# 10XGenomics/vartrix

Hardware: NVIDIA H100
Metric: reads_sw_scored_per_sec (higher is better)
Workload: dtype int16x2

## Files before the change

### include/vartrix_b200.h

```cpp
#ifndef VARTRIX_B200_H
#define VARTRIX_B200_H

#include <stdint.h>

#ifdef __cplusplus
extern "C" {
#endif

#define VTX_ABI_VERSION 2

#define VTX_OK             0
#define VTX_E_INVALID     (-1)
#define VTX_E_CUDA        (-2)
#define VTX_E_NOMEM       (-3)
#define VTX_E_UNSUPPORTED (-4)
#define VTX_E_STATE       (-5)
#define VTX_E_NCCL        (-6)

#define VTX_MODE_CONSENSUS 0
#define VTX_MODE_COVERAGE  1
#define VTX_MODE_ALT_FRAC  2

#define VTX_NO_CB   0xFFFFFFFFu
#define VTX_NO_UMI  0xFFFFFFFFFFFFFFFFull
// ... 162 lines not shown
int         vtx_submit_bam(vtx_ctx* ctx, const vtx_bam_shard* shard);
int         vtx_bam_metrics_get(vtx_ctx* ctx, vtx_bam_metrics* out);
int         vtx_set_min_base_quality(vtx_ctx* ctx, uint32_t min_q);
int         vtx_bam_low_base_quality(vtx_ctx* ctx, uint64_t* out);

uint64_t    vtx_pack_cb(const uint8_t* s, uint32_t len);

typedef struct vtx_timing {
    float h2d_ms;
    float prep_ms;
    float sw_ms;
    float post_ms;
    uint64_t n_pairs;
    uint64_t sw_launches;
    uint64_t total_launches;
} vtx_timing;
int         vtx_last_timing(vtx_ctx* ctx, vtx_timing* out);
int         vtx_last_tile_counts(vtx_ctx* ctx, uint32_t* out, uint32_t n_out);

int         vtx_comm_unique_id(uint8_t id_out[128]);
int         vtx_comm_init(vtx_ctx* ctx, const uint8_t id[128], int32_t rank, int32_t n_ranks);
int         vtx_gather(vtx_ctx* ctx, vtx_result* out);
#define VTX_GATHER_ALL (-1)
int         vtx_gather_start(vtx_ctx* ctx, int32_t root);
int         vtx_gather_wait(vtx_ctx* ctx, vtx_result* out);

#ifdef __cplusplus
}
#endif
#endif
// ... 1 lines not shown
```

### vartrix_b200/_capi.py

```python
from __future__ import annotations

import ctypes as C
import os

_HERE = os.path.dirname(os.path.abspath(__file__))
LIB_PATH = os.environ.get("VTX_LIB") or os.path.join(_HERE, "lib", "libvartrix_b200.so")

VTX_OK = 0
MODE_CONSENSUS, MODE_COVERAGE, MODE_ALT_FRAC = 0, 1, 2
MODES = {"consensus": MODE_CONSENSUS, "coverage": MODE_COVERAGE, "alt_frac": MODE_ALT_FRAC}
NO_CB = 0xFFFFFFFF
NO_UMI = 0xFFFFFFFFFFFFFFFF
F_KEEP_SCORES = 1
F_NO_SPLIT = 2
F_VALUES_ONLY = 4
F_NO_FOLD = 8
F_NAME_KEYS = 16

SYMBOLS = [
    "vtx_abi_version", "vtx_create", "vtx_destroy", "vtx_last_error", "vtx_host_alloc", "vtx_host_free",
    "vtx_set_barcodes", "vtx_submit", "vtx_submit_device", "vtx_submit_device_ex", "vtx_finish",
    "vtx_finish_device", "vtx_fetch", "vtx_sync", "vtx_wait_copies", "vtx_score_pairs", "vtx_pack_umi", "vtx_last_timing", "vtx_last_tile_counts",
    "vtx_comm_unique_id", "vtx_comm_init", "vtx_gather", "vtx_gather_start", "vtx_gather_wait",
    "vtx_submit2", "vtx_submit2_device", "vtx_pack_cb", "vtx_bgzf_inflate", "vtx_submit_bam", "vtx_bam_metrics_get",
# ... 61 lines not shown
                ("num_duplicates", C.c_uint64), ("num_not_useful", C.c_uint64)]


class Metrics(C.Structure):
    _fields_ = [("num_not_cell_bc", C.c_uint64), ("num_non_umi", C.c_uint64), ("num_scored", C.c_uint64)]


class Result(C.Structure):
    _fields_ = [("n", C.c_uint64), ("row", C.c_void_p), ("col", C.c_void_p), ("ref_cnt", C.c_void_p),
                ("alt_cnt", C.c_void_p), ("unk_cnt", C.c_void_p), ("val", C.c_void_p), ("val2", C.c_void_p),
                ("metrics", Metrics)]


class Timing(C.Structure):
    _fields_ = [("h2d_ms", C.c_float), ("prep_ms", C.c_float), ("sw_ms", C.c_float), ("post_ms", C.c_float),
                ("n_pairs", C.c_uint64), ("sw_launches", C.c_uint64), ("total_launches", C.c_uint64)]


_lib = None


def load():
    global _lib
    if _lib is not None:
        return _lib
    if not os.path.exists(LIB_PATH):
        raise RuntimeError(f"{LIB_PATH} is missing: run `make` (or __graft_entry__.build()) first; "
                           "vartrix_b200 has no CPU fallback")
    L = C.CDLL(LIB_PATH)
    L.vtx_abi_version.restype = C.c_int
    L.vtx_create.restype = C.c_int
# ... 58 lines not shown
```

### vartrix_b200/csrc/vtx_api.cu

```cuda
#include "../../include/vartrix_b200.h"
#include "vtx_pipeline.cuh"
#include "vtx_sw.cuh"
#include "vtx_sw_band.cuh"
#include "vtx_inflate.cuh"
#include "vtx_stage.cuh"

#include <nvtx3/nvToolsExt.h>

#include <algorithm>
#include <array>
#include <cstdarg>
#include <cstddef>
#include <cstdio>
#include <cstring>
#include <string>
#include <thread>
#include <vector>

using namespace vtx;

namespace {

thread_local std::string g_create_error;

// ... 88 lines not shown
    DBuf inf_comp, inf_out, inf_desc, inf_status;
    bool inflate_attr_set = false;
    StageSlot sslot[2];
    uint64_t n_bam_submits = 0;
    cudaStream_t stage_stream = nullptr;
    DBuf bam_metrics;
    uint32_t min_base_quality = 0;
    DBuf stage_sums;
    HostBuf h_stage;
    uint32_t bc_cap = 0, n_barcodes = 0;
    bool have_barcodes = false;

    InSlot slot[2];
    uint64_t n_submits = 0;
    cudaStream_t copy_stream = nullptr;
    DBuf read_col, keep, pidx, scan_sums, pair_read, pair_col, pair_umi, pair_locus, pair_start, tcount, tstart,
        pair_first, pair_cslot, pair_uslot, cslot_col, cslot_locus, uslot_cslot, ccnt, ucnt, keep2, oidx, tile_counters,
        scratch, pair_scores, d_metrics, d_res_n, big_list, slot_scratch;
    DBuf res[kResArrays];
    size_t res_cap = 0;
    size_t res_ub = 0;
    bool finished = true;
    HostResults h_res;
    HostBuf h_scalars;
    uint64_t last_n = 0;
    vtx_metrics last_metrics{};

    cudaStream_t fetch_stream = nullptr;
    HostBuf h_cum;
    unsigned long long* d_cum = nullptr;
    std::vector<TimeRec> trecs;
    size_t trec_used = 0;
    bool timing_valid = false;
    uint32_t last_tiles_nl = 0;
    bool last_tiles_valid = false;
    uint64_t t_pairs = 0;

    void* comm = nullptr;
    int rank = 0, n_ranks = 1;
    HostResults g_host;
    DBuf g_dev[kResArrays];
    DBuf g_counts;
    cudaStream_t comm_stream = nullptr;
    cudaEvent_t ev_counts = nullptr, ev_gather = nullptr, ev_results = nullptr;
    HostBuf h_counts;
    bool gather_pending = false;
    bool gather_guard = false;
    vtx_result g_out{};
};

namespace {
// ... 164 lines not shown
    return launch_sw(ctx, vtx_k_sw_pairs<CLS>, TileClass<CLS>::THREADS,
                     sw_warp_bytes<CLS>(a.mcap, a.multi) * (TileClass<CLS>::THREADS / 32), a, launches,
                     "SW kernel class", CLS);
}
template <int SCLS> int launch_sw_split(vtx_ctx* ctx, const SwArgs& a, uint64_t* launches)
{
    return launch_sw(ctx, vtx_k_sw_split<SCLS>, SplitClass<SCLS>::THREADS,
                     split_warp_bytes<SCLS>(a.mcap) * (SplitClass<SCLS>::THREADS / 32), a, launches,
                     "split SW kernel", SCLS);
}
template <int W, int S, bool SHARED> int launch_sw_fold(vtx_ctx* ctx, const SwArgs& a, uint64_t* launches)
{
    return launch_sw(ctx, vtx_k_sw_fold<W, S, SHARED>, W * 32, fold_cta_bytes<W, S>(), a, launches, "folded SW kernel", -1);
}

int run_sw(vtx_ctx* ctx, const DevBatch& b, uint32_t n_pairs_ub, const uint32_t* pair_slot, uint32_t* counters,
           uint32_t* pair_scores, uint64_t* launches, uint64_t* sw_launches, TimeRec* tr)
{
    const uint32_t nl = b.n_loci;
    ENS(ctx->tcount, size_t(kNumClasses) * (nl + 1) * 4);
    ENS(ctx->tstart, size_t(kNumClasses) * (nl + 1) * 4);
    ENS(ctx->tile_counters, 64);
    const SwAllow allow = sw_allow(ctx, b.max_read_len, b.max_hap_len);
    vtx_k_locus_prep<<<blocks_for(uint64_t(nl) * 32, 256), 256, 0, ctx->stream>>>(
        nl, b.hap, b.ref_off, b.ref_len, b.alt_off, b.alt_len, P<uint32_t>(ctx->pair_start), P<uint32_t>(ctx->pair_read), b.read_len,
        0, allow.split, allow.multi, allow.fold, b.max_read_len, b.max_hap_len, P<unsigned long long>(ctx->d_metrics) + 4,
        P<uint32_t>(ctx->tcount));
    ++*launches;
    vtx_k_scan_rows<<<kNumClasses, kScanThreads, 0, ctx->stream>>>(P<uint32_t>(ctx->tcount), P<uint32_t>(ctx->tstart), nl, nl + 1);
    ++*launches;
    CK(cudaGetLastError());
    CK(cudaMemsetAsync(ctx->tile_counters.p, 0, 64, ctx->stream));
    ctx->last_tiles_nl = nl;
    ctx->last_tiles_valid = true;
    if (tr) CK(cudaEventRecord(tr->ev[EV_PREP], ctx->stream));

    SwArgs a{};
    a.hap_bytes = b.hap; a.ref_off = b.ref_off; a.ref_len = b.ref_len; a.alt_off = b.alt_off; a.alt_len = b.alt_len;
    a.read_nib = b.read_nib; a.read_off = b.read_off; a.read_len = b.read_len;
    a.pair_read = P<uint32_t>(ctx->pair_read); a.pair_start = P<uint32_t>(ctx->pair_start);
    a.n_loci = nl; a.pair_slot = pair_slot; a.counters = counters; a.pair_scores = pair_scores;
    a.min_score = ctx->cfg.min_score;
    int mcap = int(std::min<uint32_t>(b.max_read_len, kFastMaxRead));
    mcap = std::max(2, (mcap + 1) & ~1);
    a.mcap = mcap;
    a.k64k = 65536u;
    a.one = 1u;
    a.multi = allow.multi;
    a.max_hap = b.max_hap_len;

    uint64_t before = *launches;
    if (ctx->cfg.band_mode == VTX_BAND_MODEL) {
        BandArgs ba{};
        ba.sw = a; ba.n_pairs_ub = n_pairs_ub; ba.k = ctx->cfg.band_k; ba.w = ctx->cfg.band_w;
        ba.max_read = std::max<uint32_t>(b.max_read_len, 8); ba.max_hap = std::max<uint32_t>(b.max_hap_len, 8);
// ... 86 lines not shown
    }
    ctx->res_cap = ncap;
    return VTX_OK;
}

int process_batch(vtx_ctx* ctx, const DevBatch& b, TimeRec* tr)
{
    const uint64_t nc = b.n_cand;
    const uint32_t nl = b.n_loci, nr = b.n_reads;
    const int use_umi = ctx->cfg.use_umi ? 1 : 0;
    uint64_t launches = 0, sw_launches = 0;
    cudaStream_t st = ctx->stream;

    if (ctx->finished) {
        CK(cudaMemsetAsync(ctx->d_res_n.p, 0, 8, st));
        CK(cudaMemsetAsync(ctx->d_metrics.p, 0, 48, st));
        ctx->res_ub = 0;
        ctx->finished = false;
    }
    int rc = grow_results(ctx, ctx->res_ub + nc);
    if (rc) return rc;

    const size_t ncp = size_t(nc) + 1;
    ENS(ctx->read_col, size_t(nr ? nr : 1) * 4);
    ENS(ctx->keep, ncp * 4); ENS(ctx->pidx, ncp * 4);
    ENS(ctx->pair_read, ncp * 4); ENS(ctx->pair_col, ncp * 4);
    if (use_umi) ENS(ctx->pair_umi, ncp * 8);
    ENS(ctx->pair_start, size_t(nl + 1) * 4);
    ENS(ctx->pair_first, ncp);
    ENS(ctx->pair_cslot, ncp * 4); ENS(ctx->cslot_col, ncp * 4); ENS(ctx->cslot_locus, ncp * 4);
    ENS(ctx->ccnt, ncp * 16);
// ... 865 lines not shown
}

int vtx_wait_copies(vtx_ctx* ctx)
{
    if (!ctx) return VTX_E_INVALID;
    CK(cudaSetDevice(ctx->device));
    CK(cudaStreamSynchronize(ctx->copy_stream));
    return VTX_OK;
}

static int finish_scalars(vtx_ctx* ctx)
{
    CK(cudaSetDevice(ctx->device));
    uint64_t* hs = ctx->h_scalars.as<uint64_t>();
    CK(cudaMemcpyAsync(hs, ctx->d_res_n.p, 8, cudaMemcpyDeviceToHost, ctx->stream));
    CK(cudaMemcpyAsync(hs + 1, ctx->d_metrics.p, 48, cudaMemcpyDeviceToHost, ctx->stream));
    CK(cudaStreamSynchronize(ctx->stream));
    const uint64_t violated = ctx->finished ? 0 : hs[5], band_overflow = ctx->finished ? 0 : hs[6];
    ctx->last_n = ctx->finished ? 0 : hs[0];
    ctx->last_metrics.num_not_cell_bc = ctx->finished ? 0 : hs[1];
    ctx->last_metrics.num_non_umi = ctx->finished ? 0 : hs[2];
    ctx->last_metrics.num_scored = ctx->finished ? 0 : hs[3];
    ctx->t_pairs = ctx->last_metrics.num_scored;
    ctx->finished = true;
    if (band_overflow)
        return set_err(ctx, VTX_E_UNSUPPORTED, "band model: %llu alignments had more k-mer hits than the work buffers hold (reads x windows too large); "
                                               "they were scored with the full matrix", (unsigned long long)band_overflow);
    if (violated)
        return set_err(ctx, VTX_E_INVALID, "%llu loci of a device batch exceeded the bounds given to vtx_submit_device(_ex) (longest read / widest "
                                           "haplotype window); they were skipped, the result is incomplete", (unsigned long long)violated);
    return VTX_OK;
}

int vtx_finish_device(vtx_ctx* ctx, vtx_result* out)
{
    Nvtx nvtx_range("vtx_finish_device");
    if (!ctx || !out) return VTX_E_INVALID;
    int rc = finish_scalars(ctx);
// ... 78 lines not shown
    if (!ctx || !t) return VTX_E_INVALID;
    if (!ctx->timing_valid || ctx->trec_used == 0) return set_err(ctx, VTX_E_STATE, "no finished submit to time");
    CK(cudaSetDevice(ctx->device));
    memset(t, 0, sizeof(*t));
    for (size_t i = 0; i < ctx->trec_used; ++i) {
        TimeRec& r = ctx->trecs[i];
        CK(cudaEventSynchronize(r.ev[EV_POST]));
        float ms = 0;
        if (r.had_h2d) { CK(cudaEventElapsedTime(&ms, r.ev[EV_START], r.ev[EV_H2D])); t->h2d_ms += ms; }
        CK(cudaEventElapsedTime(&ms, r.ev[EV_C0], r.ev[EV_PREP])); t->prep_ms += ms;
        CK(cudaEventElapsedTime(&ms, r.ev[EV_PREP], r.ev[EV_SW])); t->sw_ms += ms;
        CK(cudaEventElapsedTime(&ms, r.ev[EV_SW], r.ev[EV_POST])); t->post_ms += ms;
        t->sw_launches += r.sw_launches; t->total_launches += r.launches;
    }
    t->n_pairs = ctx->t_pairs;
    return VTX_OK;
}

int vtx_score_pairs(vtx_ctx* ctx, const vtx_batch* hb, uint64_t n_pairs, const uint32_t* pair_read,
                    const uint32_t* pair_locus, int16_t* ref_score, int16_t* alt_score)
{
    Nvtx nvtx_range("vtx_score_pairs");
    if (!ctx) return VTX_E_INVALID;
    if (!hb) return set_err(ctx, VTX_E_INVALID, "batch is NULL");
    BatchView hv0 = view_of(hb); hv0.n_cand = 0; hv0.cand_read = nullptr;
    int rc = validate_batch(ctx, hv0);
    if (rc) return rc;
    if (n_pairs >= 0xFFFFFFF0ull) return set_err(ctx, VTX_E_INVALID, "too many pairs");
    if (n_pairs && (!pair_read || !pair_locus || !ref_score || !alt_score)) return set_err(ctx, VTX_E_INVALID, "NULL pair arrays");
    DevBatch d{};
// ... 225 lines not shown
```

### vartrix_b200/csrc/vtx_pipeline.cuh

```cuda
#pragma once
#include <cstdint>
#include <cuda_runtime.h>
#include "vtx_sw.cuh"
#include "vtx_sw_split.cuh"
#include "vtx_sw_fold.cuh"

namespace vtx {

constexpr uint32_t kNoCb = 0xFFFFFFFFu;
constexpr uint64_t kNoUmi = 0xFFFFFFFFFFFFFFFFull;
constexpr uint32_t kInvalid = 0xFFFFFFFFu;

__host__ __device__ inline uint64_t fnv1a64(const uint8_t* p, uint32_t n)
{
    uint64_t h = 1469598103934665603ull;
    for (uint32_t i = 0; i < n; ++i) { h ^= p[i]; h *= 1099511628211ull; }
    return h;
}

struct BarcodeTable {
    const int32_t* slot;
    uint32_t cap_mask;
    const uint8_t* bytes;
    const uint32_t* off;
// ... 158 lines not shown
{
    const uint32_t l = blockIdx.x * blockDim.x + threadIdx.x;
    if (l <= n_loci) pair_start[l] = pidx[cand_start[l]];
}

__global__ void vtx_k_pair_start_explicit(uint32_t n_loci, uint32_t n_pairs, const uint32_t* __restrict__ pair_locus,
                                          uint32_t* __restrict__ pair_start)
{
    const uint32_t l = blockIdx.x * blockDim.x + threadIdx.x;
    if (l > n_loci) return;
    uint32_t lo = 0, hi = n_pairs;
    while (lo < hi) { const uint32_t mid = (lo + hi) >> 1; if (pair_locus[mid] < l) lo = mid + 1; else hi = mid; }
    pair_start[l] = lo;
}

__global__ void vtx_k_locus_prep(uint32_t n_loci, const uint8_t* __restrict__ hap_bytes,
                                 const uint32_t* __restrict__ ref_off, const uint32_t* __restrict__ ref_len,
                                 const uint32_t* __restrict__ alt_off, const uint32_t* __restrict__ alt_len,
                                 const uint32_t* __restrict__ pair_start, const uint32_t* __restrict__ pair_read,
                                 const uint32_t* __restrict__ read_len, int force_slow, int allow_split, int allow_multi, int allow_fold,
                                 uint32_t max_read, uint32_t max_hap, unsigned long long* __restrict__ bounds_violated,
                                 uint32_t* __restrict__ tcount )
{
    const uint32_t l = (blockIdx.x * blockDim.x + threadIdx.x) >> 5;
    const int lane = threadIdx.x & 31;
    if (l >= n_loci) return;
    const uint32_t nr = ref_len[l], na = alt_len[l];
    const uint8_t* rh = hap_bytes + ref_off[l];
    const uint8_t* ah = hap_bytes + alt_off[l];
    bool exotic = false;
    auto is_exotic = [](uint8_t b) {
        return b == '=' || b == 'M' || b == 'R' || b == 'S' || b == 'V' || b == 'W' || b == 'Y' || b == 'H' ||
               b == 'K' || b == 'D' || b == 'B' || b == 'N';
    };
    for (uint32_t j = lane; j < nr; j += 32) exotic |= is_exotic(rh[j]);
    for (uint32_t j = lane; j < na; j += 32) exotic |= is_exotic(ah[j]);
    exotic = __any_sync(0xffffffffu, exotic);
    bool same = nr >= uint32_t(kSplitP) && na >= uint32_t(kSplitP);
    if (same) for (uint32_t j = lane; j < uint32_t(kSplitP); j += 32) same &= (rh[j] == ah[j]);
    same = __all_sync(0xffffffffu, same);
    bool fold = same && allow_fold && min(nr, na) > uint32_t(2 * kFoldP) && max(nr, na) <= uint32_t(2 * kFoldP + kFoldMaxMid);
    if (fold) for (uint32_t j = lane; j < uint32_t(kFoldP); j += 32) fold &= (rh[nr - 1 - j] == ah[na - 1 - j]);
    fold = __all_sync(0xffffffffu, fold);
    uint32_t longest = 0;
    for (uint32_t p = pair_start[l] + lane; p < pair_start[l + 1]; p += 32) longest = max(longest, read_len[pair_read[p]]);
    longest = __reduce_max_sync(0xffffffffu, longest);
    fold = fold && longest <= uint32_t(kFoldMaxRead);
    if (lane != 0) return;
    const uint32_t nmax = max(nr, na);
    if (longest > max_read || nmax > max_hap) {
        atomicAdd(bounds_violated, 1ull);
#pragma unroll
        for (int c = 0; c < kNumClasses; ++c) tcount[size_t(c) * (n_loci + 1) + l] = 0u;
        return;
    }
    int cls = kSlowClass;
    if (!exotic && !force_slow) {
#pragma unroll
        for (int c = kNumFastClasses - 1; c >= 0; --c) if (nmax <= uint32_t(class_max_n(c))) cls = c;
        if (cls == kSlowClass && allow_multi) cls = kMultiClass;
        if (same && allow_split) {
#pragma unroll
            for (int c = kNumSplitClasses - 1; c >= 0; --c) if (nmax <= uint32_t(split_max_n(c))) cls = kSplitClass0 + c;
        }
        if (fold) cls = kFoldClass;
    }
    const uint32_t np = pair_start[l + 1] - pair_start[l];
#pragma unroll
    for (int c = 0; c < kNumClasses; ++c) {
        const uint32_t ppw = (c == kSlowClass) ? uint32_t(kSlowPairsPerWarp) : (c == kFoldClass ? uint32_t(kFoldPPW) : (c > kSlowClass ? uint32_t(kSplitPPW) : 4u));
        tcount[size_t(c) * (n_loci + 1) + l] = (c == cls) ? (np + ppw - 1) / ppw : 0u;
    }
}

constexpr int kSlotThreads = 128;
constexpr int kSlotChunk = 1024;
constexpr uint32_t kSlotSmallMax = 2048;
constexpr int kSlotBigThreads = 1024;
constexpr int kSlotBigWords = 7;
__global__ void __launch_bounds__(kSlotThreads) vtx_k_slots(
    uint32_t n_loci, const uint32_t* __restrict__ pair_start, const uint32_t* __restrict__ pair_col,
    const uint64_t* __restrict__ pair_umi, int use_umi, uint8_t* __restrict__ pair_first,
// ... 326 lines not shown
```

### vartrix_b200/csrc/vtx_sw.cuh

```cuda
#pragma once
#include <cstdint>
#include <cuda_runtime.h>

namespace vtx {

constexpr int kMatch = 1, kMismatch = -5, kGapOpen = -5, kGapExtend = -1;
constexpr int kGoe = kGapOpen + kGapExtend;

__host__ __device__ constexpr uint32_t pack2(int lo, int hi)
{
    return (uint32_t(uint16_t(int16_t(hi))) << 16) | uint32_t(uint16_t(int16_t(lo)));
}
constexpr int kBias = 16384;
constexpr uint32_t kGE2 = pack2(kGapExtend, kGapExtend);
constexpr uint32_t kBIAS2 = pack2(kBias, kBias);
constexpr uint32_t kGOE2 = pack2(kBias + kGoe, kBias + kGoe);
constexpr uint32_t kNEG2 = pack2(0, 0);
constexpr uint32_t kGoeAdd = (uint32_t(uint16_t(int16_t(kGoe - 1))) << 16) | uint32_t(uint16_t(int16_t(kGoe)));
#ifndef VTX_SW_FUSE
#define VTX_SW_FUSE 1
#endif
#ifndef VTX_SW_HADD
#define VTX_SW_HADD 0
#endif
// ... 42 lines not shown
template <> struct TileClass<3> { static constexpr int LPP = 8, C = 40, CS = 44, THREADS = 384, MINB = 1; };
constexpr int kMultiClass = 3;
constexpr int kMultiMaxRead = 256;
__host__ __device__ constexpr int class_max_n(int cls)
{
    return cls == 0 ? 208 : cls == 1 ? 232 : cls == 2 ? 256 : cls == 3 ? 320 : 0x7fffffff;
}
constexpr int kSlowPairsPerWarp = 16;

struct SwArgs {
    const uint8_t* hap_bytes;
    const uint32_t* ref_off; const uint32_t* ref_len; const uint32_t* alt_off; const uint32_t* alt_len;
    const uint8_t* read_nib; const uint64_t* read_off; const uint32_t* read_len;
    const uint32_t* pair_read;
    const uint32_t* pair_start;
    const uint32_t* tile_start;
    uint32_t n_loci;
    uint32_t* tile_counter;
    const uint32_t* pair_slot;
    uint32_t* counters;
    uint32_t* pair_scores;
    int32_t min_score;
    int32_t mcap;
    uint32_t k64k;
    uint32_t one;
    int32_t multi;
    uint32_t* scratch;
    uint32_t max_hap;
};

// ... 4 lines not shown
__device__ __forceinline__ uint32_t nib_code(uint32_t nib)
{
    return (0x4444444344424104ull >> (nib * 4)) & 0xF;
}

__device__ __forceinline__ uint32_t upper_locus(const uint32_t* __restrict__ a, uint32_t n, uint32_t v)
{
    uint32_t lo = 0, hi = n;
    while (hi - lo > 1) {
        uint32_t mid = (lo + hi) >> 1;
        if (__ldg(a + mid) <= v) lo = mid; else hi = mid;
    }
    return lo;
}

__device__ __forceinline__ void call_and_scatter(const SwArgs& a, uint32_t pair, uint32_t packed)
{
    const int ref_score = int(int16_t(packed & 0xFFFF)), alt_score = int(int16_t(packed >> 16));
    if (a.pair_scores) a.pair_scores[pair] = pack2(ref_score, alt_score);
    if (!a.pair_slot) return;
    if (ref_score < a.min_score && alt_score < a.min_score) return;
    const uint32_t k = ref_score > alt_score ? 0u : (alt_score > ref_score ? 1u : 2u);
    atomicAdd(a.counters + size_t(a.pair_slot[pair]) * 4 + k, 1u);
}

template <int CLS>
__host__ __device__ constexpr size_t sw_warp_bytes(int mcap, int multi)
{
    using TC = TileClass<CLS>;
    constexpr int PPW = 32 / TC::LPP, RS = TC::LPP * TC::CS;
    const int bnd_stride = (CLS == kMultiClass && multi) ? mcap + 8 : 0;
    const size_t codes_bytes = (size_t(PPW) * (mcap + 2 * TC::LPP) * 2 + 7) & ~size_t(7);
    return (size_t(5 * RS) * 4 + codes_bytes + size_t(PPW) * bnd_stride * 8 + 15) & ~size_t(15);
}

template <int CLS>
__global__ void __launch_bounds__(TileClass<CLS>::THREADS, TileClass<CLS>::MINB) vtx_k_sw_pairs(const SwArgs a)
{
// ... 23 lines not shown
    uint32_t cached_locus = 0xFFFFFFFFu;
    const uint32_t tile_chunk = max(1u, min(uint32_t(kTileChunk), n_tiles / (gridDim.x * (blockDim.x >> 5) * 16u)));

    for (;;) {
        uint32_t chunk = 0;
        if (lane == 0) chunk = atomicAdd(a.tile_counter, 1u);
        chunk = __shfl_sync(0xffffffffu, chunk, 0);
        const uint32_t t_begin = chunk * tile_chunk;
        if (t_begin >= n_tiles) break;
        const uint32_t t_end = min(t_begin + tile_chunk, n_tiles);

        uint32_t locus = upper_locus(a.tile_start, a.n_loci, t_begin);
        for (uint32_t tile = t_begin; tile < t_end; ++tile) {
            while (tile >= __ldg(a.tile_start + locus + 1)) ++locus;
            const uint32_t p0 = __ldg(a.pair_start + locus) + PPW * (tile - __ldg(a.tile_start + locus));
            const uint32_t p_end = __ldg(a.pair_start + locus + 1);

            __syncwarp();
            const uint8_t* rh = a.hap_bytes + __ldg(a.ref_off + locus);
            const uint8_t* ah = a.hap_bytes + __ldg(a.alt_off + locus);
            const int n_ref = int(__ldg(a.ref_len + locus)), n_alt = int(__ldg(a.alt_len + locus));
            const int n_pass = MULTI ? max(1, (max(n_ref, n_alt) + LPP * C - 1) / (LPP * C)) : 1;
            auto build_profile = [&](int col0) {
                for (int idx = lane; idx < RS; idx += 32) {
                    const int gg = idx / CS, k = idx - gg * CS;
                    const int j = col0 + gg * C + k;
                    uint32_t rb = 5, ab = 5;
                    if (k < C) {
                        if (j < n_ref) rb = hap_code(__ldg(rh + j));
                        if (j < n_alt) ab = hap_code(__ldg(ah + j));
                    }
// ... 96 lines not shown

__global__ void __launch_bounds__(128) vtx_k_sw_generic(const SwArgs a)
{
    const int lane = threadIdx.x & 31;
    const uint32_t gwarp = (blockIdx.x * blockDim.x + threadIdx.x) >> 5;
    uint32_t* rowbuf = a.scratch + size_t(gwarp) * (size_t(a.max_hap) + 1) * 32 + lane;
    const uint32_t n_tiles = __ldg(a.tile_start + a.n_loci);
    const int sub = lane >> 1, which = lane & 1;
    for (;;) {
        uint32_t tile = 0;
        if (lane == 0) tile = atomicAdd(a.tile_counter, 1u);
        tile = __shfl_sync(0xffffffffu, tile, 0);
        if (tile >= n_tiles) break;
        const uint32_t locus = upper_locus(a.tile_start, a.n_loci, tile);
        const uint32_t p0 = __ldg(a.pair_start + locus) + kSlowPairsPerWarp * (tile - __ldg(a.tile_start + locus));
        const uint32_t p_end = __ldg(a.pair_start + locus + 1);
        const uint32_t pair = p0 + sub;
        int score = 0;
        if (pair < p_end) {
            const uint32_t r = __ldg(a.pair_read + pair);
            const int m = int(__ldg(a.read_len + r));
            const uint8_t* nib = a.read_nib + __ldg(a.read_off + r);
            const uint8_t* hap = a.hap_bytes + (which ? __ldg(a.alt_off + locus) : __ldg(a.ref_off + locus));
            const int n = int(which ? __ldg(a.alt_len + locus) : __ldg(a.ref_len + locus));
            for (int j = 0; j <= n; ++j) rowbuf[size_t(j) * 32] = pack2(0, -30000);
            for (int i = 0; i < m; ++i) {
                const uint32_t by = __ldg(nib + (i >> 1));
                const uint8_t xc = uint8_t("=ACMGRSVTWYHKDBN"[(i & 1) ? (by & 0xF) : (by >> 4)]);
                int diag = 0, left = 0, e = -30000;
                for (int j = 1; j <= n; ++j) {
                    const uint32_t w = rowbuf[size_t(j) * 32];
// ... 20 lines not shown
```

### vartrix_b200/csrc/vtx_sw_fold.cuh

```cuda
#pragma once
#include <cuda/atomic>
#include "vtx_sw.cuh"
#include "vtx_fold_ring.cuh"

namespace vtx {

constexpr int kFoldP = 96;
constexpr int kFoldC1 = 12;
constexpr int kFoldPPW = 4;
constexpr int kFoldR = 19;
constexpr int kFoldMaxRead = 8 * kFoldR;
constexpr int kFoldMaxMid = 40;
constexpr int kFoldRows = kFoldMaxRead + 4;
constexpr int kFoldCodeStride = kFoldMaxRead + 16;
constexpr int kFoldPairRows = 25;
#ifndef VTX_FOLD_UNROLL
#define VTX_FOLD_UNROLL 4
#endif
constexpr int kFoldDeepWarps = 20, kFoldDeepSlots = 9;
constexpr int kFoldShallowWarps = 13;
#ifndef VTX_FOLD_DEEP_DEPTH
#define VTX_FOLD_DEEP_DEPTH 6
#endif
constexpr uint32_t kFoldDeepDepth = VTX_FOLD_DEEP_DEPTH;
// ... 88 lines not shown
        } else {
            if (w_next == w_end) {
                uint32_t chunk = 0;
                if (lane == 0) chunk = atomicAdd(a.tile_counter, 1u);
                chunk = __shfl_sync(0xffffffffu, chunk, 0);
                w_next = chunk * run_len;
                if (w_next >= n_tiles) break;
                w_end = min(w_next + run_len, n_tiles);
                w_locus = upper_locus(a.tile_start, a.n_loci, w_next);
            }
            tile = w_next++;
            while (tile >= __ldg(a.tile_start + w_locus + 1)) ++w_locus;
            locus = w_locus;
            slot = warp;
            build = locus != w_cached;
            w_cached = locus;
        }
        const uint32_t p0 = __ldg(a.pair_start + locus) + kFoldPPW * (tile - __ldg(a.tile_start + locus));
        const uint32_t p_end = __ldg(a.pair_start + locus + 1);
        uint32_t* prof = reinterpret_cast<uint32_t*>(slots + slot * kFoldSlotBytes);
        uint32_t* midtab = prof + kFoldPairRows * RS1;
        if (build) {
            const uint8_t* rh = a.hap_bytes + __ldg(a.ref_off + locus);
            const uint8_t* ah = a.hap_bytes + __ldg(a.alt_off + locus);
            const int n_ref = int(__ldg(a.ref_len + locus)), n_alt = int(__ldg(a.alt_len + locus));
            const int mid_ref = n_ref - 2 * P, mid_alt = n_alt - 2 * P;
            if (lane == 0) ring.mids[slot] = uint32_t(mid_ref) | uint32_t(mid_alt) << 16;
            if (lane < P / 4) {
                uint32_t fb[4], sb[4];
#pragma unroll
                for (int k = 0; k < 4; ++k) {
                    fb[k] = hap_code(__ldg(rh + 4 * lane + k));
                    sb[k] = hap_code(__ldg(rh + (n_ref - 1 - 4 * lane - k)));
                }
// ... 6 lines not shown
                        for (int k = 0; k < 4; ++k)
                            w[k] = pack2(ra == fb[k] ? kProfMatch : kProfMis, rb == sb[k] ? kProfMatch : kProfMis);
                        reinterpret_cast<uint4*>(prof + (5 * ra + rb) * RS1)[lane] = make_uint4(w[0], w[1], w[2], w[3]);
                    }
            }
            const int lmax = max(mid_ref, mid_alt);
            for (int idx = lane; idx < lmax * 8; idx += 32) {
                const int k = idx >> 3;
                const uint32_t r = uint32_t(idx & 7);
                const uint32_t rb = k < mid_ref ? hap_code(__ldg(rh + P + k)) : 5u;
                const uint32_t ab = k < mid_alt ? hap_code(__ldg(ah + P + k)) : 5u;
                midtab[idx] = pack2(r == rb ? kProfMatch : kProfMis, r == ab ? kProfMatch : kProfMis);
            }
            __syncwarp();
            if (SHARED && lane == 0) ring_publish<FoldSyncDev>(ring, slot);
        } else if (SHARED) {
            ring_wait<FoldSyncDev>(ring, slot);
        }
        const int mid_ref = int(ring.mids[slot] & 0xFFFFu), mid_alt = int(ring.mids[slot] >> 16);
        const uint32_t pair = p0 + u;
        const bool active = pair < p_end;
        int m = 0;
        uint8_t* cf = codes + (2 * u) * kFoldCodeStride;
        uint8_t* cp = cf + kFoldCodeStride;
        {
            const uint8_t* nib = nullptr;
            if (active) {
                const uint32_t rd = __ldg(a.pair_read + pair);
                m = int(__ldg(a.read_len + rd));
                nib = a.read_nib + __ldg(a.read_off + rd);
            }
            for (int e = g; e < kFoldCodeStride; e += 8)
// ... 145 lines not shown
```

### vartrix_b200/csrc/vtx_sw_split.cuh

```cuda
#pragma once
#include "vtx_sw.cuh"

namespace vtx {

constexpr int kSplitP = 96;
constexpr int kSplitC1 = 12;
constexpr int kSplitPPW = 8;
constexpr int kSplitMaxRead = 256;

template <int SCLS> struct SplitClass;
#ifndef VTX_SPLIT0_COPIES
#define VTX_SPLIT0_COPIES 1
#endif
#ifndef VTX_SPLIT0_THREADS
#define VTX_SPLIT0_THREADS 320
#endif
#ifndef VTX_SPLIT1_COPIES
#define VTX_SPLIT1_COPIES 1
#endif
#ifndef VTX_SPLIT_ONLY
#define VTX_SPLIT_ONLY 0
#endif
#ifndef VTX_SPLIT1_THREADS
#define VTX_SPLIT1_THREADS 256
// ... 42 lines not shown
    const uint32_t tile_chunk = max(1u, min(uint32_t(kTileChunk), n_tiles / (gridDim.x * (blockDim.x >> 5) * 16u)));
    const uint32_t k64k = a.k64k;
    const uint32_t one = a.one;

    for (;;) {
        uint32_t chunk = 0;
        if (lane == 0) chunk = atomicAdd(a.tile_counter, 1u);
        chunk = __shfl_sync(0xffffffffu, chunk, 0);
        const uint32_t t_begin = chunk * tile_chunk;
        if (t_begin >= n_tiles) break;
        const uint32_t t_end = min(t_begin + tile_chunk, n_tiles);
        uint32_t locus = upper_locus(a.tile_start, a.n_loci, t_begin);
        for (uint32_t tile = t_begin; tile < t_end; ++tile) {
            while (tile >= __ldg(a.tile_start + locus + 1)) ++locus;
            const uint32_t p0 = __ldg(a.pair_start + locus) + kSplitPPW * (tile - __ldg(a.tile_start + locus));
            const uint32_t p_end = __ldg(a.pair_start + locus + 1);
            __syncwarp();
            if (locus != cached_locus) {
                cached_locus = locus;
                const uint8_t* rh = a.hap_bytes + __ldg(a.ref_off + locus);
                const uint8_t* ah = a.hap_bytes + __ldg(a.alt_off + locus);
                const int n_ref = int(__ldg(a.ref_len + locus)), n_alt = int(__ldg(a.alt_len + locus));
                for (int j = lane; j < P; j += 32) {
                    const uint32_t rb = hap_code(__ldg(rh + j));
#pragma unroll
                    for (uint32_t r = 0; r < 5; ++r) {
                        prof1[r * RS1 + j] = uint32_t(r == rb ? kProfMatch : kProfMis);
                    }
                }
                for (int idx = lane; idx < 4 * CS2; idx += 32) {
                    const int gg = idx / CS2, k = idx - gg * CS2;
// ... 164 lines not shown
```

### vartrix_b200/engine.py

```python
from __future__ import annotations

import ctypes as C
from dataclasses import dataclass, field

import numpy as np

from . import _capi

MODES = _capi.MODES
NO_CB, NO_UMI = _capi.NO_CB, _capi.NO_UMI


class VtxError(RuntimeError):
    pass


_FIELDS = ("locus_row", "hap_bytes", "ref_off", "ref_len", "alt_off", "alt_len", "cand_start", "read_nib",
           "read_off", "read_len", "cb_bytes", "read_cb_off", "read_cb_len", "read_umi_key", "cand_read")
_DTYPES = dict(locus_row=np.uint32, hap_bytes=np.uint8, ref_off=np.uint32, ref_len=np.uint32, alt_off=np.uint32,
               alt_len=np.uint32, cand_start=np.uint64, read_nib=np.uint8, read_off=np.uint64, read_len=np.uint32,
               cb_bytes=np.uint8, read_cb_off=np.uint32, read_cb_len=np.uint16, read_umi_key=np.uint64,
               cand_read=np.uint32)


# ... 399 lines not shown
        return self._triplets(res, copy)

    def finish_device(self) -> _capi.Result:
        res = _capi.Result()
        self._ck(self._L.vtx_finish_device(self._h, C.byref(res)), "vtx_finish_device")
        self._keep.clear()
        return res

    def sync(self):
        self._ck(self._L.vtx_sync(self._h), "vtx_sync")

    def timing(self) -> dict:
        t = _capi.Timing()
        self._ck(self._L.vtx_last_timing(self._h, C.byref(t)), "vtx_last_timing")
        return dict(h2d_ms=t.h2d_ms, prep_ms=t.prep_ms, sw_ms=t.sw_ms, post_ms=t.post_ms, n_pairs=int(t.n_pairs),
                    sw_launches=int(t.sw_launches), total_launches=int(t.total_launches))

    def tile_counts(self) -> list:
        out = (C.c_uint32 * 16)()
        n = self._L.vtx_last_tile_counts(self._h, out, 16)
        if n < 0:
            self._ck(n, "vtx_last_tile_counts")
        return [int(out[i]) for i in range(n)]

    def run(self, batch: StagedBatch) -> Triplets:
        self.submit(batch)
        return self.finish()

    def score_pairs(self, batch: StagedBatch, pair_read, pair_locus):
        pr = np.ascontiguousarray(pair_read, np.uint32); pl = np.ascontiguousarray(pair_locus, np.uint32)
        rs = np.zeros(len(pr), np.int16); as_ = np.zeros(len(pr), np.int16)
# ... 115 lines not shown
```

Before: 160.0 million.

## Resolve exact-substring reads in locus prep and skip their Smith-Waterman

```diff
diff --git a/include/vartrix_b200.h b/include/vartrix_b200.h
--- a/include/vartrix_b200.h
+++ b/include/vartrix_b200.h
@@ -200,6 +200,7 @@
     uint64_t n_pairs;
     uint64_t sw_launches;
     uint64_t total_launches;
+    uint64_t n_exact;
 } vtx_timing;
 int         vtx_last_timing(vtx_ctx* ctx, vtx_timing* out);
 int         vtx_last_tile_counts(vtx_ctx* ctx, uint32_t* out, uint32_t n_out);
diff --git a/vartrix_b200/_capi.py b/vartrix_b200/_capi.py
--- a/vartrix_b200/_capi.py
+++ b/vartrix_b200/_capi.py
@@ -99,7 +99,8 @@
 
 class Timing(C.Structure):
     _fields_ = [("h2d_ms", C.c_float), ("prep_ms", C.c_float), ("sw_ms", C.c_float), ("post_ms", C.c_float),
-                ("n_pairs", C.c_uint64), ("sw_launches", C.c_uint64), ("total_launches", C.c_uint64)]
+                ("n_pairs", C.c_uint64), ("sw_launches", C.c_uint64), ("total_launches", C.c_uint64),
+                ("n_exact", C.c_uint64)]
 
 
 _lib = None
diff --git a/vartrix_b200/csrc/vtx_api.cu b/vartrix_b200/csrc/vtx_api.cu
--- a/vartrix_b200/csrc/vtx_api.cu
+++ b/vartrix_b200/csrc/vtx_api.cu
@@ -126,7 +126,7 @@
     InSlot slot[2];
     uint64_t n_submits = 0;
     cudaStream_t copy_stream = nullptr;
-    DBuf read_col, keep, pidx, scan_sums, pair_read, pair_col, pair_umi, pair_locus, pair_start, tcount, tstart,
+    DBuf read_col, keep, pidx, scan_sums, pair_read, pair_col, pair_umi, pair_locus, pair_start, pair_end, tcount, tstart,
         pair_first, pair_cslot, pair_uslot, cslot_col, cslot_locus, uslot_cslot, ccnt, ucnt, keep2, oidx, tile_counters,
         scratch, pair_scores, d_metrics, d_res_n, big_list, slot_scratch;
     DBuf res[kResArrays];
@@ -147,6 +147,7 @@
     uint32_t last_tiles_nl = 0;
     bool last_tiles_valid = false;
     uint64_t t_pairs = 0;
+    uint64_t t_exact = 0;
 
     void* comm = nullptr;
     int rank = 0, n_ranks = 1;
@@ -341,7 +342,7 @@
     return launch_sw(ctx, vtx_k_sw_fold<W, S, SHARED>, W * 32, fold_cta_bytes<W, S>(), a, launches, "folded SW kernel", -1);
 }
 
-int run_sw(vtx_ctx* ctx, const DevBatch& b, uint32_t n_pairs_ub, const uint32_t* pair_slot, uint32_t* counters,
+int run_sw(vtx_ctx* ctx, const DevBatch& b, uint32_t n_pairs_ub, uint32_t* pair_slot, uint32_t* counters,
            uint32_t* pair_scores, uint64_t* launches, uint64_t* sw_launches, TimeRec* tr)
 {
     const uint32_t nl = b.n_loci;
@@ -349,10 +350,17 @@
     ENS(ctx->tstart, size_t(kNumClasses) * (nl + 1) * 4);
     ENS(ctx->tile_counters, 64);
     const SwAllow allow = sw_allow(ctx, b.max_read_len, b.max_hap_len);
-    vtx_k_locus_prep<<<blocks_for(uint64_t(nl) * 32, 256), 256, 0, ctx->stream>>>(
-        nl, b.hap, b.ref_off, b.ref_len, b.alt_off, b.alt_len, P<uint32_t>(ctx->pair_start), P<uint32_t>(ctx->pair_read), b.read_len,
-        0, allow.split, allow.multi, allow.fold, b.max_read_len, b.max_hap_len, P<unsigned long long>(ctx->d_metrics) + 4,
-        P<uint32_t>(ctx->tcount));
+    ExactArgs ex{};
+    const bool exact = pair_slot && !pair_scores && ctx->cfg.band_mode != VTX_BAND_MODEL;
+    if (exact) {
+        ENS(ctx->pair_end, size_t(nl) * 4 + 4);
+        ex.pair_end = P<uint32_t>(ctx->pair_end); ex.pair_slot = pair_slot; ex.counters = counters;
+        ex.min_score = ctx->cfg.min_score; ex.n_exact = P<unsigned long long>(ctx->d_metrics) + 6;
+    }
+    vtx_k_locus_prep<<<blocks_for(uint64_t(nl) * 32, kPrepThreads), kPrepThreads, 0, ctx->stream>>>(
+        nl, b.hap, b.ref_off, b.ref_len, b.alt_off, b.alt_len, P<uint32_t>(ctx->pair_start), P<uint32_t>(ctx->pair_read),
+        b.read_nib, b.read_off, b.read_len, 0, allow.split, allow.multi, allow.fold, b.max_read_len, b.max_hap_len,
+        P<unsigned long long>(ctx->d_metrics) + 4, ex, P<uint32_t>(ctx->tcount));
     ++*launches;
     vtx_k_scan_rows<<<kNumClasses, kScanThreads, 0, ctx->stream>>>(P<uint32_t>(ctx->tcount), P<uint32_t>(ctx->tstart), nl, nl + 1);
     ++*launches;
@@ -366,6 +374,7 @@
     a.hap_bytes = b.hap; a.ref_off = b.ref_off; a.ref_len = b.ref_len; a.alt_off = b.alt_off; a.alt_len = b.alt_len;
     a.read_nib = b.read_nib; a.read_off = b.read_off; a.read_len = b.read_len;
     a.pair_read = P<uint32_t>(ctx->pair_read); a.pair_start = P<uint32_t>(ctx->pair_start);
+    a.pair_end = exact ? P<uint32_t>(ctx->pair_end) : P<uint32_t>(ctx->pair_start) + 1;
     a.n_loci = nl; a.pair_slot = pair_slot; a.counters = counters; a.pair_scores = pair_scores;
     a.min_score = ctx->cfg.min_score;
     int mcap = int(std::min<uint32_t>(b.max_read_len, kFastMaxRead));
@@ -482,7 +491,7 @@
 
     if (ctx->finished) {
         CK(cudaMemsetAsync(ctx->d_res_n.p, 0, 8, st));
-        CK(cudaMemsetAsync(ctx->d_metrics.p, 0, 48, st));
+        CK(cudaMemsetAsync(ctx->d_metrics.p, 0, 56, st));
         ctx->res_ub = 0;
         ctx->finished = false;
     }
@@ -1378,7 +1387,7 @@
     CK(cudaSetDevice(ctx->device));
     uint64_t* hs = ctx->h_scalars.as<uint64_t>();
     CK(cudaMemcpyAsync(hs, ctx->d_res_n.p, 8, cudaMemcpyDeviceToHost, ctx->stream));
-    CK(cudaMemcpyAsync(hs + 1, ctx->d_metrics.p, 48, cudaMemcpyDeviceToHost, ctx->stream));
+    CK(cudaMemcpyAsync(hs + 1, ctx->d_metrics.p, 56, cudaMemcpyDeviceToHost, ctx->stream));
     CK(cudaStreamSynchronize(ctx->stream));
     const uint64_t violated = ctx->finished ? 0 : hs[5], band_overflow = ctx->finished ? 0 : hs[6];
     ctx->last_n = ctx->finished ? 0 : hs[0];
@@ -1386,6 +1395,7 @@
     ctx->last_metrics.num_non_umi = ctx->finished ? 0 : hs[2];
     ctx->last_metrics.num_scored = ctx->finished ? 0 : hs[3];
     ctx->t_pairs = ctx->last_metrics.num_scored;
+    ctx->t_exact = ctx->finished ? 0 : hs[7];
     ctx->finished = true;
     if (band_overflow)
         return set_err(ctx, VTX_E_UNSUPPORTED, "band model: %llu alignments had more k-mer hits than the work buffers hold (reads x windows too large); "
@@ -1494,6 +1504,7 @@
         t->sw_launches += r.sw_launches; t->total_launches += r.launches;
     }
     t->n_pairs = ctx->t_pairs;
+    t->n_exact = ctx->t_exact;
     return VTX_OK;
 }
 
diff --git a/vartrix_b200/csrc/vtx_pipeline.cuh b/vartrix_b200/csrc/vtx_pipeline.cuh
--- a/vartrix_b200/csrc/vtx_pipeline.cuh
+++ b/vartrix_b200/csrc/vtx_pipeline.cuh
@@ -196,14 +196,121 @@
     pair_start[l] = lo;
 }
 
-__global__ void vtx_k_locus_prep(uint32_t n_loci, const uint8_t* __restrict__ hap_bytes,
-                                 const uint32_t* __restrict__ ref_off, const uint32_t* __restrict__ ref_len,
-                                 const uint32_t* __restrict__ alt_off, const uint32_t* __restrict__ alt_len,
-                                 const uint32_t* __restrict__ pair_start, const uint32_t* __restrict__ pair_read,
-                                 const uint32_t* __restrict__ read_len, int force_slow, int allow_split, int allow_multi, int allow_fold,
-                                 uint32_t max_read, uint32_t max_hap, unsigned long long* __restrict__ bounds_violated,
-                                 uint32_t* __restrict__ tcount )
-{
+constexpr int kPrepThreads = 256;
+constexpr uint32_t kExactMaxHap = 512;
+constexpr uint32_t kExactMaxRead = 256;
+constexpr uint32_t kExactMaxDepth = 2048;
+constexpr int kExactHapWords = int(kExactMaxHap) / 16 + 2;
+constexpr int kExactReadWords = int(kExactMaxRead) / 16;
+
+struct ExactArgs {
+    uint32_t* pair_end;
+    uint32_t* pair_slot;
+    uint32_t* counters;
+    int32_t min_score;
+    unsigned long long* n_exact;
+};
+
+__device__ __forceinline__ void load16(const uint8_t* __restrict__ p, uint32_t have, uint32_t fill, uint32_t (&w)[4])
+{
+    if (have >= 16 && (reinterpret_cast<uintptr_t>(p) & 15) == 0) {
+        const uint4 v = __ldg(reinterpret_cast<const uint4*>(p));
+        w[0] = v.x; w[1] = v.y; w[2] = v.z; w[3] = v.w;
+        return;
+    }
+#pragma unroll
+    for (int q = 0; q < 4; ++q) {
+        w[q] = 0;
+#pragma unroll
+        for (int b = 0; b < 4; ++b) w[q] |= (uint32_t(4 * q + b) < have ? uint32_t(__ldg(p + 4 * q + b)) : fill) << (8 * b);
+    }
+}
+
+__device__ __forceinline__ void exact_pack_hap(const uint8_t* __restrict__ h, uint32_t n, uint32_t* code, uint32_t* valid, int lane)
+{
+    const uint32_t nw = (n + 15) / 16 + 1;
+    for (uint32_t w = lane; w < nw; w += 32) {
+        uint32_t by[4], c = 0, v = 0;
+        load16(h + 16 * w, 16 * w < n ? n - 16 * w : 0u, 0u, by);
+#pragma unroll
+        for (int i = 0; i < 16; ++i) {
+            const uint32_t hc = hap_code(uint8_t(by[i >> 2] >> (8 * (i & 3))));
+            if (hc < 4) { c |= hc << (2 * i); v |= 1u << i; }
+        }
+        code[w] = c; valid[w] = v;
+    }
+}
+
+__device__ __forceinline__ uint32_t nib8_codes(uint32_t x, bool& ok)
+{
+    uint32_t p = x - ((x >> 1) & 0x55555555u);
+    p = (p & 0x33333333u) + ((p >> 2) & 0x33333333u);
+    ok &= p == 0x11111111u;
+    const uint32_t c = ((x >> 1) & 0x77777777u) - ((x >> 3) & 0x11111111u);
+    uint32_t t = ((c >> 4) & 0x03030303u) | ((c & 0x03030303u) << 2);
+    t = (t | (t >> 4)) & 0x00FF00FFu;
+    return (t | (t >> 8)) & 0x0000FFFFu;
+}
+
+__device__ __forceinline__ bool exact_pack_read(const uint8_t* __restrict__ nib, uint32_t m, uint32_t* rw)
+{
+    const uint32_t nbytes = (m + 1) / 2;
+    const uint32_t pad_q = (m & 1) ? (nbytes - 1) / 4 : 0xFFFFFFFFu, pad_s = 8 * ((nbytes - 1) & 3);
+    bool ok = true;
+    for (uint32_t j = 0; 16 * j < nbytes; ++j) {
+        uint32_t by[4];
+        load16(nib + 16 * j, nbytes - 16 * j, 0x11u, by);
+#pragma unroll
+        for (int q = 0; q < 4; ++q)
+            if (4 * j + q == pad_q) by[q] = (by[q] & ~(0xFu << pad_s)) | (1u << pad_s);
+#pragma unroll
+        for (int h = 0; h < 2; ++h)
+            if (32 * j + 16 * h < m) rw[32 * (2 * j + h)] = nib8_codes(by[2 * h], ok) | nib8_codes(by[2 * h + 1], ok) << 16;
+    }
+    return ok;
+}
+
+__device__ __forceinline__ bool exact_occurs(const uint32_t* code, const uint32_t* valid, uint32_t n, const uint32_t* rw, uint32_t m)
+{
+    if (m > n) return false;
+    const uint32_t r0 = rw[0];
+    const uint32_t cm0 = m >= 16 ? 0xFFFFFFFFu : (1u << (2 * m)) - 1;
+    const uint32_t nwr = (m + 15) / 16, last = n - m;
+    for (uint32_t w = 0; 16 * w <= last; ++w) {
+        const uint32_t lo = code[w], hi = code[w + 1];
+        uint32_t hits = 0;
+#pragma unroll
+        for (int s = 0; s < 16; ++s) hits |= uint32_t(((__funnelshift_r(lo, hi, 2 * s) ^ r0) & cm0) == 0) << s;
+        hits &= last - 16 * w >= 15 ? 0xFFFFu : (2u << (last - 16 * w)) - 1;
+        while (hits) {
+            const uint32_t o = 16 * w + __ffs(hits) - 1;
+            hits &= hits - 1;
+            bool ok = true;
+            for (uint32_t k = 0; k < nwr && ok; ++k) {
+                const uint32_t p = o + 16 * k, pw = p >> 4, ps = p & 15, nb = min(m - 16 * k, 16u);
+                const uint32_t cm = nb == 16 ? 0xFFFFFFFFu : (1u << (2 * nb)) - 1, vm = (1u << nb) - 1;
+                const uint32_t c = __funnelshift_r(code[pw], code[pw + 1], 2 * ps);
+                const uint32_t v = (valid[pw] | (valid[pw + 1] << 16)) >> ps;
+                ok = ((c ^ rw[32 * k]) & cm) == 0 && (v & vm) == vm;
+            }
+            if (ok) return true;
+        }
+    }
+    return false;
+}
+
+__global__ void __launch_bounds__(kPrepThreads) vtx_k_locus_prep(
+    uint32_t n_loci, const uint8_t* __restrict__ hap_bytes,
+    const uint32_t* __restrict__ ref_off, const uint32_t* __restrict__ ref_len,
+    const uint32_t* __restrict__ alt_off, const uint32_t* __restrict__ alt_len,
+    const uint32_t* __restrict__ pair_start, uint32_t* __restrict__ pair_read,
+    const uint8_t* __restrict__ read_nib, const uint64_t* __restrict__ read_off,
+    const uint32_t* __restrict__ read_len, int force_slow, int allow_split, int allow_multi, int allow_fold,
+    uint32_t max_read, uint32_t max_hap, unsigned long long* __restrict__ bounds_violated, ExactArgs ex,
+    uint32_t* __restrict__ tcount )
+{
+    __shared__ uint32_t s_code[kPrepThreads / 32][2][kExactHapWords], s_valid[kPrepThreads / 32][2][kExactHapWords];
+    __shared__ uint32_t s_read[kPrepThreads / 32][kExactReadWords * 32];
     const uint32_t l = (blockIdx.x * blockDim.x + threadIdx.x) >> 5;
     const int lane = threadIdx.x & 31;
     if (l >= n_loci) return;
@@ -224,13 +331,54 @@
     bool fold = same && allow_fold && min(nr, na) > uint32_t(2 * kFoldP) && max(nr, na) <= uint32_t(2 * kFoldP + kFoldMaxMid);
     if (fold) for (uint32_t j = lane; j < uint32_t(kFoldP); j += 32) fold &= (rh[nr - 1 - j] == ah[na - 1 - j]);
     fold = __all_sync(0xffffffffu, fold);
+    const uint32_t ps = pair_start[l], pe = pair_start[l + 1];
     uint32_t longest = 0;
-    for (uint32_t p = pair_start[l] + lane; p < pair_start[l + 1]; p += 32) longest = max(longest, read_len[pair_read[p]]);
+    for (uint32_t p = ps + lane; p < pe; p += 32) longest = max(longest, read_len[pair_read[p]]);
     longest = __reduce_max_sync(0xffffffffu, longest);
     fold = fold && longest <= uint32_t(kFoldMaxRead);
+    const uint32_t nmax = max(nr, na);
+    const bool violated = longest > max_read || nmax > max_hap;
+    if (ex.pair_end) {
+        uint32_t kept = pe;
+        if (!violated && nmax <= kExactMaxHap) {
+            const int w = threadIdx.x >> 5;
+            exact_pack_hap(rh, nr, s_code[w][0], s_valid[w][0], lane);
+            exact_pack_hap(ah, na, s_code[w][1], s_valid[w][1], lane);
+            __syncwarp();
+            uint32_t* rw = s_read[w] + lane;
+            kept = ps;
+            for (uint32_t base = ps; base < pe; base += 32) {
+                const uint32_t p = base + lane;
+                uint32_t rd = 0, slot = 0;
+                bool undecided = false;
+                if (p < pe) {
+                    rd = pair_read[p];
+                    slot = ex.pair_slot[p];
+                    const uint32_t m = read_len[rd];
+                    bool ok = base - ps < kExactMaxDepth && m >= 1 && m <= kExactMaxRead;
+                    if (ok) {
+                        ok = exact_pack_read(read_nib + read_off[rd], m, rw);
+                    }
+                    const bool in_ref = ok && exact_occurs(s_code[w][0], s_valid[w][0], nr, rw, m);
+                    const bool in_alt = ok && exact_occurs(s_code[w][1], s_valid[w][1], na, rw, m);
+                    if (in_ref || in_alt) count_call(ex.counters, slot, ex.min_score, int(m) - !in_ref, int(m) - !in_alt);
+                    else undecided = true;
+                }
+                __syncwarp();
+                const uint32_t bal = __ballot_sync(0xffffffffu, undecided);
+                if (undecided) {
+                    const uint32_t d = kept + __popc(bal & ((1u << lane) - 1u));
+                    pair_read[d] = rd;
+                    ex.pair_slot[d] = slot;
+                }
+                kept += __popc(bal);
+            }
+            if (lane == 0 && kept < pe) atomicAdd(ex.n_exact, (unsigned long long)(pe - kept));
+        }
+        if (lane == 0) ex.pair_end[l] = kept;
+    }
     if (lane != 0) return;
-    const uint32_t nmax = max(nr, na);
-    if (longest > max_read || nmax > max_hap) {
+    if (violated) {
         atomicAdd(bounds_violated, 1ull);
 #pragma unroll
         for (int c = 0; c < kNumClasses; ++c) tcount[size_t(c) * (n_loci + 1) + l] = 0u;
@@ -247,7 +395,7 @@
         }
         if (fold) cls = kFoldClass;
     }
-    const uint32_t np = pair_start[l + 1] - pair_start[l];
+    const uint32_t np = pe - ps;
 #pragma unroll
     for (int c = 0; c < kNumClasses; ++c) {
         const uint32_t ppw = (c == kSlowClass) ? uint32_t(kSlowPairsPerWarp) : (c == kFoldClass ? uint32_t(kFoldPPW) : (c > kSlowClass ? uint32_t(kSplitPPW) : 4u));
diff --git a/vartrix_b200/csrc/vtx_sw.cuh b/vartrix_b200/csrc/vtx_sw.cuh
--- a/vartrix_b200/csrc/vtx_sw.cuh
+++ b/vartrix_b200/csrc/vtx_sw.cuh
@@ -80,6 +80,7 @@
     const uint8_t* read_nib; const uint64_t* read_off; const uint32_t* read_len;
     const uint32_t* pair_read;
     const uint32_t* pair_start;
+    const uint32_t* pair_end;
     const uint32_t* tile_start;
     uint32_t n_loci;
     uint32_t* tile_counter;
@@ -114,14 +115,18 @@
     return lo;
 }
 
+__device__ __forceinline__ void count_call(uint32_t* counters, uint32_t slot, int min_score, int ref_score, int alt_score)
+{
+    if (ref_score < min_score && alt_score < min_score) return;
+    const uint32_t k = ref_score > alt_score ? 0u : (alt_score > ref_score ? 1u : 2u);
+    atomicAdd(counters + size_t(slot) * 4 + k, 1u);
+}
 __device__ __forceinline__ void call_and_scatter(const SwArgs& a, uint32_t pair, uint32_t packed)
 {
     const int ref_score = int(int16_t(packed & 0xFFFF)), alt_score = int(int16_t(packed >> 16));
     if (a.pair_scores) a.pair_scores[pair] = pack2(ref_score, alt_score);
     if (!a.pair_slot) return;
-    if (ref_score < a.min_score && alt_score < a.min_score) return;
-    const uint32_t k = ref_score > alt_score ? 0u : (alt_score > ref_score ? 1u : 2u);
-    atomicAdd(a.counters + size_t(a.pair_slot[pair]) * 4 + k, 1u);
+    count_call(a.counters, a.pair_slot[pair], a.min_score, ref_score, alt_score);
 }
 
 template <int CLS>
@@ -175,7 +180,8 @@
         for (uint32_t tile = t_begin; tile < t_end; ++tile) {
             while (tile >= __ldg(a.tile_start + locus + 1)) ++locus;
             const uint32_t p0 = __ldg(a.pair_start + locus) + PPW * (tile - __ldg(a.tile_start + locus));
-            const uint32_t p_end = __ldg(a.pair_start + locus + 1);
+            const uint32_t p_end = __ldg(a.pair_end + locus);
+            if (p0 >= p_end) continue;
 
             __syncwarp();
             const uint8_t* rh = a.hap_bytes + __ldg(a.ref_off + locus);
@@ -302,7 +308,8 @@
         if (tile >= n_tiles) break;
         const uint32_t locus = upper_locus(a.tile_start, a.n_loci, tile);
         const uint32_t p0 = __ldg(a.pair_start + locus) + kSlowPairsPerWarp * (tile - __ldg(a.tile_start + locus));
-        const uint32_t p_end = __ldg(a.pair_start + locus + 1);
+        const uint32_t p_end = __ldg(a.pair_end + locus);
+        if (p0 >= p_end) continue;
         const uint32_t pair = p0 + sub;
         int score = 0;
         if (pair < p_end) {
diff --git a/vartrix_b200/csrc/vtx_sw_fold.cuh b/vartrix_b200/csrc/vtx_sw_fold.cuh
--- a/vartrix_b200/csrc/vtx_sw_fold.cuh
+++ b/vartrix_b200/csrc/vtx_sw_fold.cuh
@@ -126,10 +126,14 @@
             locus = w_locus;
             slot = warp;
             build = locus != w_cached;
+        }
+        const uint32_t p0 = __ldg(a.pair_start + locus) + kFoldPPW * (tile - __ldg(a.tile_start + locus));
+        const uint32_t p_end = __ldg(a.pair_end + locus);
+        const bool empty = p0 >= p_end;
+        if (!SHARED) {
+            if (empty) continue;
             w_cached = locus;
         }
-        const uint32_t p0 = __ldg(a.pair_start + locus) + kFoldPPW * (tile - __ldg(a.tile_start + locus));
-        const uint32_t p_end = __ldg(a.pair_start + locus + 1);
         uint32_t* prof = reinterpret_cast<uint32_t*>(slots + slot * kFoldSlotBytes);
         uint32_t* midtab = prof + kFoldPairRows * RS1;
         if (build) {
@@ -166,8 +170,12 @@
             }
             __syncwarp();
             if (SHARED && lane == 0) ring_publish<FoldSyncDev>(ring, slot);
-        } else if (SHARED) {
+        } else if (SHARED && !empty) {
             ring_wait<FoldSyncDev>(ring, slot);
+        }
+        if (SHARED && empty) {
+            if (lane == 0) ring_release<FoldSyncDev>(ring, slot);
+            continue;
         }
         const int mid_ref = int(ring.mids[slot] & 0xFFFFu), mid_alt = int(ring.mids[slot] >> 16);
         const uint32_t pair = p0 + u;
diff --git a/vartrix_b200/csrc/vtx_sw_split.cuh b/vartrix_b200/csrc/vtx_sw_split.cuh
--- a/vartrix_b200/csrc/vtx_sw_split.cuh
+++ b/vartrix_b200/csrc/vtx_sw_split.cuh
@@ -80,7 +80,8 @@
         for (uint32_t tile = t_begin; tile < t_end; ++tile) {
             while (tile >= __ldg(a.tile_start + locus + 1)) ++locus;
             const uint32_t p0 = __ldg(a.pair_start + locus) + kSplitPPW * (tile - __ldg(a.tile_start + locus));
-            const uint32_t p_end = __ldg(a.pair_start + locus + 1);
+            const uint32_t p_end = __ldg(a.pair_end + locus);
+            if (p0 >= p_end) continue;
             __syncwarp();
             if (locus != cached_locus) {
                 cached_locus = locus;
diff --git a/vartrix_b200/engine.py b/vartrix_b200/engine.py
--- a/vartrix_b200/engine.py
+++ b/vartrix_b200/engine.py
@@ -437,7 +437,7 @@
         t = _capi.Timing()
         self._ck(self._L.vtx_last_timing(self._h, C.byref(t)), "vtx_last_timing")
         return dict(h2d_ms=t.h2d_ms, prep_ms=t.prep_ms, sw_ms=t.sw_ms, post_ms=t.post_ms, n_pairs=int(t.n_pairs),
-                    sw_launches=int(t.sw_launches), total_launches=int(t.total_launches))
+                    sw_launches=int(t.sw_launches), total_launches=int(t.total_launches), n_exact=int(t.n_exact))
 
     def tile_counts(self) -> list:
         out = (C.c_uint32 * 16)()
```

New measurement: 177.0 million, median of 6. 1.11x the previous value.
